# endernewton/tf-faster-rcnn

Hardware: NVIDIA H100
Metric: images/sec (higher is better)
Workload: dtype f16x3 (fp32-grade: fp16 hi/lo split of both operands, 3 wgmma f16 MMAs per product, fp32 accumulate)

## Files before the change

tf_faster_rcnn_b200/csrc/common.cuh:

```cuda
#pragma once
#include <cuda_runtime.h>
#include <cuda.h>
#include <stdint.h>
#include <stdio.h>

namespace frcnn {

enum Status : int {
  OK = 0, ERR_CUDA = -1, ERR_ARG = -2, ERR_NO_DEVICE = -3, ERR_DRIVER_ENTRY = -4, ERR_CAPACITY = -5
};
void set_error(const char* fmt, ...);
int cuda_fail(cudaError_t e, const char* what, const char* file, int line);

#define FRCNN_CUDA(expr)                                                        \
  do {                                                                          \
    cudaError_t _e = (expr);                                                    \
    if (_e != cudaSuccess) return ::frcnn::cuda_fail(_e, #expr, __FILE__, __LINE__); \
  } while (0)

#define FRCNN_LAUNCH_CHECK() FRCNN_CUDA(cudaGetLastError())

#define FRCNN_REQUIRE(cond, ...)                    \
  do {                                              \
    if (!(cond)) {                                  \
// ... 119 lines not shown
      "%32, %33, %34, %35, %36, %37, %38, %39, %40, %41, %42, %43, %44, %45, %46, %47, "
      "%48, %49, %50, %51, %52, %53, %54, %55, %56, %57, %58, %59, %60, %61, %62, %63}, "
      "{%64, %65, %66, %67}, %68, p, 1, 1, 0;\n\t}\n"
      : "+f"(d[0]), "+f"(d[1]), "+f"(d[2]), "+f"(d[3]), "+f"(d[4]), "+f"(d[5]), "+f"(d[6]), "+f"(d[7]),
        "+f"(d[8]), "+f"(d[9]), "+f"(d[10]), "+f"(d[11]), "+f"(d[12]), "+f"(d[13]), "+f"(d[14]), "+f"(d[15]),
        "+f"(d[16]), "+f"(d[17]), "+f"(d[18]), "+f"(d[19]), "+f"(d[20]), "+f"(d[21]), "+f"(d[22]), "+f"(d[23]),
        "+f"(d[24]), "+f"(d[25]), "+f"(d[26]), "+f"(d[27]), "+f"(d[28]), "+f"(d[29]), "+f"(d[30]), "+f"(d[31]),
        "+f"(d[32]), "+f"(d[33]), "+f"(d[34]), "+f"(d[35]), "+f"(d[36]), "+f"(d[37]), "+f"(d[38]), "+f"(d[39]),
        "+f"(d[40]), "+f"(d[41]), "+f"(d[42]), "+f"(d[43]), "+f"(d[44]), "+f"(d[45]), "+f"(d[46]), "+f"(d[47]),
        "+f"(d[48]), "+f"(d[49]), "+f"(d[50]), "+f"(d[51]), "+f"(d[52]), "+f"(d[53]), "+f"(d[54]), "+f"(d[55]),
        "+f"(d[56]), "+f"(d[57]), "+f"(d[58]), "+f"(d[59]), "+f"(d[60]), "+f"(d[61]), "+f"(d[62]), "+f"(d[63])
      : "r"(a[0]), "r"(a[1]), "r"(a[2]), "r"(a[3]), "l"(b_desc), "r"(scale_d));
}
template <> __device__ __forceinline__ void wgmma_tf32_rs<64>(float (&d)[32], const uint32_t (&a)[4], uint64_t b_desc, uint32_t scale_d) {
  asm volatile(
      "{\n\t.reg .pred p;\n\tsetp.ne.b32 p, %37, 0;\n\t"
      "wgmma.mma_async.sync.aligned.m64n64k8.f32.tf32.tf32 "
      "{%0, %1, %2, %3, %4, %5, %6, %7, %8, %9, %10, %11, %12, %13, %14, %15, "
      "%16, %17, %18, %19, %20, %21, %22, %23, %24, %25, %26, %27, %28, %29, %30, %31}, "
      "{%32, %33, %34, %35}, %36, p, 1, 1;\n\t}\n"
      : "+f"(d[0]), "+f"(d[1]), "+f"(d[2]), "+f"(d[3]), "+f"(d[4]), "+f"(d[5]), "+f"(d[6]), "+f"(d[7]),
        "+f"(d[8]), "+f"(d[9]), "+f"(d[10]), "+f"(d[11]), "+f"(d[12]), "+f"(d[13]), "+f"(d[14]), "+f"(d[15]),
        "+f"(d[16]), "+f"(d[17]), "+f"(d[18]), "+f"(d[19]), "+f"(d[20]), "+f"(d[21]), "+f"(d[22]), "+f"(d[23]),
        "+f"(d[24]), "+f"(d[25]), "+f"(d[26]), "+f"(d[27]), "+f"(d[28]), "+f"(d[29]), "+f"(d[30]), "+f"(d[31])
      : "r"(a[0]), "r"(a[1]), "r"(a[2]), "r"(a[3]), "l"(b_desc), "r"(scale_d));
}
template <> __device__ __forceinline__ void wgmma_tf32_rs<128>(float (&d)[64], const uint32_t (&a)[4], uint64_t b_desc, uint32_t scale_d) {
  asm volatile(
      "{\n\t.reg .pred p;\n\tsetp.ne.b32 p, %69, 0;\n\t"
      "wgmma.mma_async.sync.aligned.m64n128k8.f32.tf32.tf32 "
      "{%0, %1, %2, %3, %4, %5, %6, %7, %8, %9, %10, %11, %12, %13, %14, %15, "
      "%16, %17, %18, %19, %20, %21, %22, %23, %24, %25, %26, %27, %28, %29, %30, %31, "
      "%32, %33, %34, %35, %36, %37, %38, %39, %40, %41, %42, %43, %44, %45, %46, %47, "
      "%48, %49, %50, %51, %52, %53, %54, %55, %56, %57, %58, %59, %60, %61, %62, %63}, "
      "{%64, %65, %66, %67}, %68, p, 1, 1;\n\t}\n"
      : "+f"(d[0]), "+f"(d[1]), "+f"(d[2]), "+f"(d[3]), "+f"(d[4]), "+f"(d[5]), "+f"(d[6]), "+f"(d[7]),
        "+f"(d[8]), "+f"(d[9]), "+f"(d[10]), "+f"(d[11]), "+f"(d[12]), "+f"(d[13]), "+f"(d[14]), "+f"(d[15]),
        "+f"(d[16]), "+f"(d[17]), "+f"(d[18]), "+f"(d[19]), "+f"(d[20]), "+f"(d[21]), "+f"(d[22]), "+f"(d[23]),
        "+f"(d[24]), "+f"(d[25]), "+f"(d[26]), "+f"(d[27]), "+f"(d[28]), "+f"(d[29]), "+f"(d[30]), "+f"(d[31]),
        "+f"(d[32]), "+f"(d[33]), "+f"(d[34]), "+f"(d[35]), "+f"(d[36]), "+f"(d[37]), "+f"(d[38]), "+f"(d[39]),
        "+f"(d[40]), "+f"(d[41]), "+f"(d[42]), "+f"(d[43]), "+f"(d[44]), "+f"(d[45]), "+f"(d[46]), "+f"(d[47]),
        "+f"(d[48]), "+f"(d[49]), "+f"(d[50]), "+f"(d[51]), "+f"(d[52]), "+f"(d[53]), "+f"(d[54]), "+f"(d[55]),
        "+f"(d[56]), "+f"(d[57]), "+f"(d[58]), "+f"(d[59]), "+f"(d[60]), "+f"(d[61]), "+f"(d[62]), "+f"(d[63])
      : "r"(a[0]), "r"(a[1]), "r"(a[2]), "r"(a[3]), "l"(b_desc), "r"(scale_d));
}
template <int R> __device__ __forceinline__ void reg_dec() { asm volatile("setmaxnreg.dec.sync.aligned.u32 %0;" ::"n"(R)); }
template <int R> __device__ __forceinline__ void reg_inc() { asm volatile("setmaxnreg.inc.sync.aligned.u32 %0;" ::"n"(R)); }
__device__ __forceinline__ uint32_t pack_f16x2_rn(float a, float b) {
  uint32_t r;
  asm("cvt.rn.f16x2.f32 %0, %1, %2;" : "=r"(r) : "f"(b), "f"(a));
  return r;
}

__device__ __forceinline__ float4 ld_nc_f4_pinned(const float* p) {
  float4 v;
  asm volatile("ld.global.nc.v4.f32 {%0, %1, %2, %3}, [%4];" : "=f"(v.x), "=f"(v.y), "=f"(v.z), "=f"(v.w) : "l"(p));
  return v;
}
__device__ __forceinline__ float2 ld_nc_f2_pinned(const float* p) {
  float2 v;
  asm volatile("ld.global.nc.v2.f32 {%0, %1}, [%2];" : "=f"(v.x), "=f"(v.y) : "l"(p));
  return v;
}
__device__ __forceinline__ float2 ld_nc_f2_pinned_if(const float* p, bool pred) {
  float2 v = make_float2(0.f, 0.f);
  asm volatile("{\n\t.reg .pred q;\n\tsetp.ne.b32 q, %3, 0;\n\t@q ld.global.nc.v2.f32 {%0, %1}, [%2];\n\t}\n"
               : "+f"(v.x), "+f"(v.y) : "l"(p), "r"((int)pred));
  return v;
}
__device__ __forceinline__ float ld_nc_f32_pinned(const float* p) {
  float v;
  asm volatile("ld.global.nc.f32 %0, [%1];" : "=f"(v) : "l"(p));
  return v;
}

__device__ __forceinline__ float4 lds_f4(uint32_t saddr) {
  float4 v;
  asm volatile("ld.shared.v4.f32 {%0, %1, %2, %3}, [%4];" : "=f"(v.x), "=f"(v.y), "=f"(v.z), "=f"(v.w) : "r"(saddr));
  return v;
}

__device__ __forceinline__ void pdl_launch_dependents() { asm volatile("griddepcontrol.launch_dependents;" ::: "memory"); }
__device__ __forceinline__ void pdl_wait() { asm volatile("griddepcontrol.wait;" ::: "memory"); }

__device__ __forceinline__ float to_tf32_fast(float x) {
  return __uint_as_float((__float_as_uint(x) + 0x1000u) & 0xffffe000u);
}

__device__ __forceinline__ float to_tf32(float x) {
  uint32_t r;
  asm("cvt.rna.tf32.f32 %0, %1;" : "=r"(r) : "f"(x));
  return __uint_as_float(r);
}

#endif
}
```

tf_faster_rcnn_b200/csrc/conv_gemm.cu:

```cuda
#include <cuda_fp16.h>
#include "common.cuh"
#include "../../include/frcnn_b200.h"
#include <stdlib.h>
#include <string.h>

namespace frcnn {

constexpr int BLOCK_M = 128;
constexpr int BLOCK_K = 32;
constexpr int A_TILE_BYTES = BLOCK_M * BLOCK_K * 4;
constexpr int NUM_CONSUMERS = 256;
constexpr int NUM_THREADS = NUM_CONSUMERS + 128;
constexpr int REGS_PRODUCER = 40, REGS_CONSUMER = 232;
constexpr int STAGES = 3;

struct ConvKernelParams {
  float* out;
  const float* residual;
  const float* scale;
  const float* shift;
  int cout, ho, wo, nimg;
  int tn, th, tw;
  int tiles_h, tiles_w;
  int kh, kw, cin, stride, pad_t, pad_l;
  int act;
  int a_box_bytes;
  int kb_per_split;
  int m_tiles, n_tiles, total_units, n_full, splits;
  int raster_n;
  float* ws;
  long long* trace;
  int num_kb_total;
};

#ifdef FRCNN_WATCHDOG
#define FRCNN_TRACE(slot, kbv)                                                              \
  do {                                                                                      \
    if (p.trace && blockIdx.x == 0 && (kbv) < 64) p.trace[(kbv) * 8 + (slot)] = clock64(); \
  } while (0)
#else
#define FRCNN_TRACE(slot, kbv) do { } while (0)
#endif

template <int MODE> struct KTraits {
  static constexpr bool TF32 = MODE == FRCNN_CONV_TF32X3;
  static constexpr bool X1 = MODE == FRCNN_CONV_F16X1;
  static constexpr int BOXES = TF32 ? 1 : 2;
  static constexpr int A_BYTES = BOXES * A_TILE_BYTES;
  static constexpr float LO_SCALE = TF32 ? 1.f : 0.00048828125f;
};
template <int BN> constexpr int b_plane_bytes() { return BN * 128; }
template <int BN, int MODE> constexpr int stage_bytes() { return KTraits<MODE>::A_BYTES + 2 * b_plane_bytes<BN>(); }
template <int BN, int MODE> constexpr int smem_bytes() {
  return STAGES * stage_bytes<BN, MODE>() + 1024  + 64 ;
}
static_assert(smem_bytes<128, FRCNN_CONV_F16X3>() <= 227 * 1024, "ring exceeds the sm_90 shared-memory limit per block");

struct Unit {
  int w0, h0, n0, nblk, z, kb0, num_kb, slot;
};
__device__ __forceinline__ Unit decode_unit(const ConvKernelParams& p, int u, int num_kb_total) {
  Unit t;
  int tile;
  if (u < p.n_full) { tile = u; t.z = 0; t.slot = -1; }
  else { const int v = u - p.n_full; t.slot = v / p.splits; t.z = v - t.slot * p.splits; tile = p.n_full + t.slot; }
  int mt;
  if (p.raster_n) { t.nblk = tile % p.n_tiles; mt = tile / p.n_tiles; }
  else { mt = tile % p.m_tiles; t.nblk = tile / p.m_tiles; }
  const int tile_w = mt % p.tiles_w;
  const int tile_h = (mt / p.tiles_w) % p.tiles_h;
  const int tile_n = mt / (p.tiles_w * p.tiles_h);
  t.w0 = tile_w * p.tw; t.h0 = tile_h * p.th; t.n0 = tile_n * p.tn;
  if (t.slot < 0) { t.kb0 = 0; t.num_kb = num_kb_total; }
  else { t.kb0 = t.z * p.kb_per_split; t.num_kb = min(p.kb_per_split, num_kb_total - t.kb0); }
  return t;
}

template <int ACT>
__device__ __forceinline__ float apply_act(float a) {
  if (ACT == FRCNN_ACT_RELU) return fmaxf(a, 0.f);
  if (ACT == FRCNN_ACT_RELU6) return fminf(fmaxf(a, 0.f), 6.f);
  return a;
}

template <bool RES, int ACT>
__device__ __forceinline__ float2 finish2(const float2 v, const float2 sc, const float2 sh, const float2 r) {
  float2 y;
  y.x = __fadd_rn(__fmul_rn(v.x, sc.x), sh.x); y.y = __fadd_rn(__fmul_rn(v.y, sc.y), sh.y);
  if (RES) { y.x = __fadd_rn(y.x, r.x); y.y = __fadd_rn(y.y, r.y); }
  y.x = apply_act<ACT>(y.x); y.y = apply_act<ACT>(y.y);
  return y;
}

constexpr int EPI_CHUNK = 8;
template <int BN, bool RES, int ACT>
__device__ __forceinline__ void epilogue_vec(const ConvKernelParams& p, const float (&acc)[BN / 2], const int cbase,
                                             const int pix0, const int pix1) {
  const int cout = p.cout;
  constexpr int NJ = BN / 8;
  constexpr int CH = NJ < EPI_CHUNK ? NJ : EPI_CHUNK;
  static_assert(NJ % CH == 0, "chunking");
  const float* const res0 = RES ? p.residual + (size_t)(pix0 >= 0 ? pix0 : 0) * cout : nullptr;
  const float* const res1 = RES ? p.residual + (size_t)(pix1 >= 0 ? pix1 : 0) * cout : nullptr;
#pragma unroll
  for (int j0 = 0; j0 < NJ; j0 += CH) {
    if (cbase + 8 * j0 >= cout) break;
    float2 sc[CH], sh[CH], r0[CH], r1[CH];
#pragma unroll
    for (int jj = 0; jj < CH; ++jj) {
      const int c = cbase + 8 * (j0 + jj);
      sc[jj] = ld_nc_f2_pinned(p.scale + c);
      sh[jj] = ld_nc_f2_pinned(p.shift + c);
      if (RES) {
        r0[jj] = ld_nc_f2_pinned_if(res0 + c, pix0 >= 0 && c < cout);
        r1[jj] = ld_nc_f2_pinned_if(res1 + c, pix1 >= 0 && c < cout);
      } else {
        r0[jj] = r1[jj] = sc[jj];
      }
    }
#pragma unroll
    for (int jj = 0; jj < CH; ++jj) {
      const int j = j0 + jj;
      const int c = cbase + 8 * j;
      if (c >= cout) break;
      if (pix0 >= 0)
        *reinterpret_cast<float2*>(p.out + (size_t)pix0 * cout + c) =
            finish2<RES, ACT>(make_float2(acc[4 * j], acc[4 * j + 1]), sc[jj], sh[jj], r0[jj]);
      if (pix1 >= 0)
        *reinterpret_cast<float2*>(p.out + (size_t)pix1 * cout + c) =
            finish2<RES, ACT>(make_float2(acc[4 * j + 2], acc[4 * j + 3]), sc[jj], sh[jj], r1[jj]);
    }
  }
}

template <int BN>
__device__ __forceinline__ void epilogue_generic(const ConvKernelParams& p, const float (&acc)[BN / 2], const int cbase,
                                                 const int pix0, const int pix1) {
#pragma unroll
  for (int j = 0; j < BN / 8; ++j) {
#pragma unroll
    for (int e = 0; e < 4; ++e) {
      const int c = cbase + 8 * j + (e & 1);
      const int pix = e < 2 ? pix0 : pix1;
      if (pix < 0 || c >= p.cout) continue;
      float a = __fadd_rn(__fmul_rn(acc[4 * j + e], p.scale[c]), p.shift[c]);
      if (p.residual) a = __fadd_rn(a, __ldg(p.residual + (size_t)pix * p.cout + c));
      if (p.act == FRCNN_ACT_RELU) a = fmaxf(a, 0.f);
      else if (p.act == FRCNN_ACT_RELU6) a = fminf(fmaxf(a, 0.f), 6.f);
      p.out[(size_t)pix * p.cout + c] = a;
    }
  }
}

template <int BN, bool RES>
__device__ __forceinline__ void epilogue_dispatch(const ConvKernelParams& p, const float (&acc)[BN / 2], const int cbase,
                                                  const int pix0, const int pix1) {
  if (p.act == FRCNN_ACT_RELU) epilogue_vec<BN, RES, FRCNN_ACT_RELU>(p, acc, cbase, pix0, pix1);
  else if (p.act == FRCNN_ACT_RELU6) epilogue_vec<BN, RES, FRCNN_ACT_RELU6>(p, acc, cbase, pix0, pix1);
  else epilogue_vec<BN, RES, FRCNN_ACT_NONE>(p, acc, cbase, pix0, pix1);
}

__device__ __forceinline__ int tile_pixel(const ConvKernelParams& p, const Unit& t, int row) {
  const int rows_img = p.th * p.tw;
  const int dn = row / rows_img, rem = row % rows_img;
  const int n = t.n0 + dn, h = t.h0 + rem / p.tw, w = t.w0 + rem % p.tw;
  const bool valid = row < p.tn * rows_img && n < p.nimg && h < p.ho && w < p.wo;
  return valid ? (int)(((long long)n * p.ho + h) * p.wo + w) : -1;
}

template <int BN>
__device__ __forceinline__ void epilogue_tile(const ConvKernelParams& p, const Unit& t, const float (&acc)[BN / 2], int r0, int q4) {
  if (t.slot >= 0) {
    float* const w = p.ws + ((size_t)t.slot * p.splits + t.z) * (size_t)(BLOCK_M * BN) + 2 * q4;
#pragma unroll
    for (int j = 0; j < BN / 8; ++j) {
      __stcg(reinterpret_cast<float2*>(w + (size_t)r0 * BN + 8 * j), make_float2(acc[4 * j], acc[4 * j + 1]));
      __stcg(reinterpret_cast<float2*>(w + (size_t)(r0 + 8) * BN + 8 * j), make_float2(acc[4 * j + 2], acc[4 * j + 3]));
    }
    return;
  }
  const int pix0 = tile_pixel(p, t, r0), pix1 = tile_pixel(p, t, r0 + 8);
  const int cbase = t.nblk * BN + 2 * q4;
  if ((p.cout & 3) != 0) {
    epilogue_generic<BN>(p, acc, cbase, pix0, pix1);
    return;
  }
  if (p.residual) epilogue_dispatch<BN, true>(p, acc, cbase, pix0, pix1);
  else epilogue_dispatch<BN, false>(p, acc, cbase, pix0, pix1);
}

template <int BN, int MODE>
__device__ __forceinline__ void wgmma_rs(float (&d)[BN / 2], const uint32_t (&a)[4], uint64_t b_desc, uint32_t scale_d) {
  if (KTraits<MODE>::TF32) wgmma_tf32_rs<BN>(d, a, b_desc, scale_d);
  else wgmma_f16_rs<BN>(d, a, b_desc, scale_d);
}

template <int BN, int MODE>
__global__ void __launch_bounds__(NUM_THREADS, 1)
conv_gemm_kernel(const __grid_constant__ CUtensorMap tmA, const __grid_constant__ CUtensorMap tmBhi,
                 const __grid_constant__ CUtensorMap tmBlo, const ConvKernelParams p) {
  using T = KTraits<MODE>;
  constexpr int kStage = stage_bytes<BN, MODE>();
  constexpr int kPlane = b_plane_bytes<BN>();
  constexpr int NACC = BN / 2;
  static_assert(BN == 64 || BN == 128, "block_n");

  extern __shared__ uint8_t smem_raw[];
  uint8_t* smem = reinterpret_cast<uint8_t*>((reinterpret_cast<uintptr_t>(smem_raw) + 1023) & ~uintptr_t(1023));
  uint64_t* full = reinterpret_cast<uint64_t*>(smem + STAGES * kStage);
  uint64_t* empty = full + STAGES;

  const int warp = threadIdx.x >> 5;
  const int lane = threadIdx.x & 31;
  const int num_kb_total = p.num_kb_total;

  if (threadIdx.x == NUM_CONSUMERS) {
    tma_prefetch_desc(&tmA); tma_prefetch_desc(&tmBhi); tma_prefetch_desc(&tmBlo);
    for (int s = 0; s < STAGES; ++s) { mbar_init(&full[s], 1); mbar_init(&empty[s], NUM_CONSUMERS); }
    mbar_fence_init();
  }
  __syncthreads();
  pdl_launch_dependents();
  pdl_wait();

  if (warp >= NUM_CONSUMERS / 32) {
    reg_dec<REGS_PRODUCER>();
    if (warp == NUM_CONSUMERS / 32 && lane == 0) {
      const int cchunks = p.cin / BLOCK_K;
      const int total32 = p.kh * p.kw * cchunks;
      const uint32_t tx = (uint32_t)(T::BOXES * p.a_box_bytes + (T::X1 ? 1 : 2) * kPlane);
      int s = 0; uint32_t ph = 0, kbt = 0;
      for (int u = blockIdx.x; u < p.total_units; u += gridDim.x) {
        const Unit t = decode_unit(p, u, num_kb_total);
#pragma unroll 1
        for (int kb = 0; kb < t.num_kb; ++kb, ++kbt) {
          MBAR_WAIT(&empty[s], ph ^ 1u, 4, kbt);
          uint8_t* st = smem + s * kStage;
          mbar_expect_tx(&full[s], tx);
#pragma unroll
          for (int i = 0; i < T::BOXES; ++i) {
            const int g32 = (t.kb0 + kb) * T::BOXES + i;
            int tap = g32 / cchunks, kc = g32 - tap * cchunks;
            if (g32 >= total32) { tap = 0; kc = cchunks; }
            const int r = tap / p.kw, sx = tap - r * p.kw;
            tma_load_4d(st + i * A_TILE_BYTES, &tmA, &full[s], kc * BLOCK_K, t.w0 * p.stride + sx - p.pad_l,
                        t.h0 * p.stride + r - p.pad_t, t.n0);
          }
          const int kcoord = (t.kb0 + kb) * T::BOXES * BLOCK_K;
          tma_load_2d(st + T::A_BYTES, &tmBhi, &full[s], kcoord, t.nblk * BN);
          if (!T::X1) tma_load_2d(st + T::A_BYTES + kPlane, &tmBlo, &full[s], kcoord, t.nblk * BN);
          FRCNN_TRACE(0, kbt);
          if (++s == STAGES) { s = 0; ph ^= 1u; }
        }
      }
    }
    return;
  }

  reg_inc<REGS_CONSUMER>();
  const int wg = warp >> 2;
  const int q4 = lane & 3;
  const int r0 = wg * 64 + (warp & 3) * 16 + (lane >> 2);
  const uint32_t swz = (uint32_t)(lane >> 2);
  uint32_t aoff[4][2];
#pragma unroll
  for (int j = 0; j < 4; ++j)
#pragma unroll
    for (int h = 0; h < 2; ++h) {
      const int ch = T::TF32 ? j * 8 + h * 4 + q4 : (j & 1) * 16 + h * 8 + 2 * q4;
      const int box = T::TF32 ? 0 : j >> 1;
      aoff[j][h] = (uint32_t)(box * A_TILE_BYTES + r0 * 128) + ((((uint32_t)ch >> 2) ^ swz) << 4) + (((uint32_t)ch & 3u) << 2);
    }
  const uint32_t smem0 = smem_u32(smem);
  int s = 0; uint32_t ph = 0, kbt = 0;
  for (int u = blockIdx.x; u < p.total_units; u += gridDim.x) {
    const Unit t = decode_unit(p, u, num_kb_total);
    float acc[NACC], part[NACC];
#pragma unroll
    for (int i = 0; i < NACC; ++i) { acc[i] = 0.f; part[i] = 0.f; }
#pragma unroll 1
    for (int kb = 0; kb < t.num_kb; ++kb, ++kbt) {
      MBAR_WAIT(&full[s], ph, 1, kbt);
      if (threadIdx.x == 0) FRCNN_TRACE(1, kbt);
      const uint32_t sa = smem0 + (uint32_t)(s * kStage);
      uint32_t ahi[4][4], alo[4][4];
#pragma unroll
      for (int j = 0; j < 4; ++j) {
#pragma unroll
        for (int f = 0; f < 4; ++f) {
          const uint32_t addr = sa + aoff[j][f >> 1] + ((f & 1) ? 1024u : 0u);
          if (T::TF32) {
            float x;
            asm volatile("ld.shared.f32 %0, [%1];" : "=f"(x) : "r"(addr));
            const float hi = to_tf32(x);
            ahi[j][f] = __float_as_uint(hi);
            alo[j][f] = __float_as_uint(to_tf32_fast(__fsub_rn(x, hi)));
          } else {
            float2 x;
            asm volatile("ld.shared.v2.f32 {%0, %1}, [%2];" : "=f"(x.x), "=f"(x.y) : "r"(addr));
            const uint32_t h = pack_f16x2_rn(x.x, x.y);
            const float2 fh = __half22float2(*reinterpret_cast<const __half2*>(&h));
            ahi[j][f] = h;
            alo[j][f] = T::X1 ? 0u : pack_f16x2_rn(__fmul_rn(__fsub_rn(x.x, fh.x), 2048.f), __fmul_rn(__fsub_rn(x.y, fh.y), 2048.f));
          }
        }
      }
      const uint64_t bhi = wgmma_sw128_desc(sa + (uint32_t)T::A_BYTES);
      const uint64_t blo = wgmma_sw128_desc(sa + (uint32_t)(T::A_BYTES + kPlane));
#pragma unroll
      for (int i = 0; i < NACC; ++i) reg_fence(part[i]);
      wgmma_fence();
#pragma unroll
      for (int j = 0; j < 4; ++j) wgmma_rs<BN, MODE>(part, ahi[j], bhi + 2u * j, j > 0 ? 1u : 0u);
      wgmma_commit();
      wgmma_wait_all();
#pragma unroll
      for (int i = 0; i < NACC; ++i) { reg_fence(part[i]); acc[i] = __fadd_rn(acc[i], part[i]); }
      if (!T::X1) {
        wgmma_fence();
#pragma unroll
        for (int j = 0; j < 4; ++j) {
          wgmma_rs<BN, MODE>(part, alo[j], bhi + 2u * j, j > 0 ? 1u : 0u);
          wgmma_rs<BN, MODE>(part, ahi[j], blo + 2u * j, 1u);
        }
        wgmma_commit();
        wgmma_wait_all();
#pragma unroll
        for (int i = 0; i < NACC; ++i) { reg_fence(part[i]); acc[i] = __fmaf_rn(part[i], T::LO_SCALE, acc[i]); }
      }
      mbar_arrive(&empty[s]);
      if (threadIdx.x == 0) FRCNN_TRACE(2, kbt);
      if (++s == STAGES) { s = 0; ph ^= 1u; }
    }
    epilogue_tile<BN>(p, t, acc, r0, q4);
  }
}

template <int BN>
__global__ void __launch_bounds__(256)
tail_reduce_kernel(const ConvKernelParams p) {
  pdl_launch_dependents();
  pdl_wait();
  constexpr int RPB = 256 / (BN / 4);
  constexpr int GROUPS = BLOCK_M / RPB;
  const int slot = blockIdx.x / GROUPS, rgroup = blockIdx.x % GROUPS;
  const int tile = p.n_full + slot;
  const int mt = p.raster_n ? tile / p.n_tiles : tile % p.m_tiles, nblk = p.raster_n ? tile % p.n_tiles : tile / p.m_tiles;
  const int tile_w = mt % p.tiles_w, tile_h = (mt / p.tiles_w) % p.tiles_h, tile_n = mt / (p.tiles_w * p.tiles_h);
  const int rows_img = p.th * p.tw;
  constexpr int C4 = BN / 4;
  static_assert(256 % C4 == 0, "each thread keeps one fixed channel group");
  const float* base = p.ws + (size_t)slot * p.splits * (size_t)(BLOCK_M * BN);
  const bool vec_ok = (p.cout & 3) == 0;
  const int cg = threadIdx.x % C4;
  const int c = nblk * BN + cg * 4;
  if (c >= p.cout) return;
  const float4 sc4 = __ldg(reinterpret_cast<const float4*>(p.scale + c)), sh4 = __ldg(reinterpret_cast<const float4*>(p.shift + c));
  const float sc[4] = {sc4.x, sc4.y, sc4.z, sc4.w}, sh[4] = {sh4.x, sh4.y, sh4.z, sh4.w};
  {
    const int row = rgroup * RPB + threadIdx.x / C4;
    const int dn = row / rows_img, rem = row % rows_img;
    const int n = tile_n * p.tn + dn, h = tile_h * p.th + rem / p.tw, w = tile_w * p.tw + rem % p.tw;
    if (row >= p.tn * rows_img || n >= p.nimg || h >= p.ho || w >= p.wo) return;
    const size_t o = ((((size_t)n * p.ho + h) * p.wo + w)) * p.cout + c;
    float4 rv = make_float4(0.f, 0.f, 0.f, 0.f);
    if (p.residual) {
      if (vec_ok) rv = __ldg(reinterpret_cast<const float4*>(p.residual + o));
      else { float t[4] = {0.f, 0.f, 0.f, 0.f}; for (int e = 0; e < 4; ++e) if (c + e < p.cout) t[e] = __ldg(p.residual + o + e); rv = make_float4(t[0], t[1], t[2], t[3]); }
    }
    float4 a = __ldg(reinterpret_cast<const float4*>(base + (size_t)row * BN) + cg);
    for (int z = 1; z < p.splits; ++z) {
      const float4 b = __ldg(reinterpret_cast<const float4*>(base + ((size_t)z * BLOCK_M + row) * BN) + cg);
      a.x = __fadd_rn(a.x, b.x); a.y = __fadd_rn(a.y, b.y); a.z = __fadd_rn(a.z, b.z); a.w = __fadd_rn(a.w, b.w);
    }
    float y[4] = {a.x, a.y, a.z, a.w};
    const float res[4] = {rv.x, rv.y, rv.z, rv.w};
#pragma unroll
    for (int e = 0; e < 4; ++e) {
      float v = y[e];
      v = __fadd_rn(__fmul_rn(v, sc[e]), sh[e]);
      if (p.residual) v = __fadd_rn(v, res[e]);
      if (p.act == FRCNN_ACT_RELU) v = fmaxf(v, 0.f);
      else if (p.act == FRCNN_ACT_RELU6) v = fminf(fmaxf(v, 0.f), 6.f);
      y[e] = v;
    }
    if (vec_ok) *reinterpret_cast<float4*>(p.out + o) = make_float4(y[0], y[1], y[2], y[3]);
    else for (int e = 0; e < 4; ++e) if (c + e < p.cout) p.out[o + e] = y[e];
// ... 1 lines not shown
}

__global__ void prep_epilogue_vectors_kernel(const float* scale, const float* shift, float out_mult, int cout, int padded,
                                             float* eff_scale, float* eff_shift) {
  const int c = blockIdx.x * blockDim.x + threadIdx.x;
  if (c >= padded) return;
  const float sc = (c < cout && scale) ? scale[c] : 1.f;
  eff_scale[c] = __fmul_rn(sc, out_mult);
  eff_shift[c] = (c < cout && shift) ? shift[c] : 0.f;
}

typedef CUresult (*EncodeTiledFn)(CUtensorMap*, CUtensorMapDataType, cuuint32_t, void*, const cuuint64_t*,
                                  const cuuint64_t*, const cuuint32_t*, const cuuint32_t*, CUtensorMapInterleave,
                                  CUtensorMapSwizzle, CUtensorMapL2promotion, CUtensorMapFloatOOBfill);

static EncodeTiledFn get_encode_fn() {
  static EncodeTiledFn fn = nullptr;
  if (!fn) {
    void* ptr = nullptr;
    cudaDriverEntryPointQueryResult qres;
    if (cudaGetDriverEntryPoint("cuTensorMapEncodeTiled", &ptr, cudaEnableDefault, &qres) == cudaSuccess &&
        qres == cudaDriverEntryPointSuccess)
      fn = reinterpret_cast<EncodeTiledFn>(ptr);
  }
  return fn;
}

static int encode_map(CUtensorMap* m, const void* base, int rank, const uint64_t* dims, const uint64_t* strides_bytes,
                      const uint32_t* box, const uint32_t* estr, CUtensorMapDataType dtype = CU_TENSOR_MAP_DATA_TYPE_FLOAT32,
                      CUtensorMapSwizzle swz = CU_TENSOR_MAP_SWIZZLE_128B) {
  EncodeTiledFn fn = get_encode_fn();
  if (!fn) { set_error("cuTensorMapEncodeTiled entry point unavailable"); return ERR_DRIVER_ENTRY; }
  cuuint64_t gd[5]; cuuint64_t gs[4]; cuuint32_t bx[5]; cuuint32_t es[5];
  for (int i = 0; i < rank; ++i) { gd[i] = dims[i]; bx[i] = box[i]; es[i] = estr[i]; }
  for (int i = 0; i + 1 < rank; ++i) gs[i] = strides_bytes[i];
  CUresult r = fn(m, dtype, (cuuint32_t)rank, const_cast<void*>(base), gd, gs, bx, es,
                  CU_TENSOR_MAP_INTERLEAVE_NONE, swz, CU_TENSOR_MAP_L2_PROMOTION_L2_256B,
                  CU_TENSOR_MAP_FLOAT_OOB_FILL_NONE);
  if (r != CUDA_SUCCESS) {
    set_error("cuTensorMapEncodeTiled failed (CUresult %d) rank=%d dims=[%llu,%llu,%llu,%llu] box=[%u,%u,%u,%u]", (int)r, rank,
              (unsigned long long)dims[0], (unsigned long long)dims[1], rank > 2 ? (unsigned long long)dims[2] : 0ull,
              rank > 3 ? (unsigned long long)dims[3] : 0ull, box[0], box[1], rank > 2 ? box[2] : 0u, rank > 3 ? box[3] : 0u);
    return ERR_CUDA;
  }
  return OK;
}

}

using namespace frcnn;

struct frcnn_conv_plan {
  CUtensorMap tmA, tmBhi, tmBlo;
  ConvKernelParams kp;
  int block_n, stages, smem;
  int impl;
  dim3 grid;
  int n_tail;
  float* ws;
  float* eff;
};

static void choose_tile(int n, int ho, int wo, int stride, int* tn, int* th, int* tw) {
  long best_tiles = -1; int bn = 1, bh = 1, bw = 1; int best_rows = 0;
  const int lim = 256 / stride;
  for (int a = 1; a <= n && a <= BLOCK_M; ++a)
    for (int b = 1; b <= ho && a * b <= BLOCK_M && b <= lim; ++b) {
      int c = BLOCK_M / (a * b);
      if (c > wo) c = wo;
      if (c > lim) c = lim;
      if (c < 1) continue;
      int tiles_w = cdiv(wo, c);
      c = cdiv(wo, tiles_w);
      long tiles = (long)cdiv(n, a) * cdiv(ho, b) * tiles_w;
      int rows = a * b * c;
      if (best_tiles < 0 || tiles < best_tiles || (tiles == best_tiles && rows < best_rows)) {
        best_tiles = tiles; bn = a; bh = b; bw = c; best_rows = rows;
      }
    }
  *tn = bn; *th = bh; *tw = bw;
}

static bool pdl_enabled() {
  static int v = -1;
  if (v < 0) { const char* e = getenv("FRCNN_NO_PDL"); v = (e && e[0] == '1') ? 0 : 1; }
  return v == 1;
}

template <int BN, int MODE>
static int launch(const frcnn_conv_plan* p, cudaStream_t st) {
  static bool attr_done = false;
  if (!attr_done) {
    FRCNN_CUDA(cudaFuncSetAttribute(conv_gemm_kernel<BN, MODE>, cudaFuncAttributeMaxDynamicSharedMemorySize, smem_bytes<BN, MODE>()));
    attr_done = true;
  }
  cudaLaunchAttribute attr[1];
  attr[0].id = cudaLaunchAttributeProgrammaticStreamSerialization;
  attr[0].val.programmaticStreamSerializationAllowed = 1;
  const bool pdl = pdl_enabled();
  cudaLaunchConfig_t cfg{};
  cfg.gridDim = p->grid; cfg.blockDim = dim3(NUM_THREADS); cfg.dynamicSmemBytes = smem_bytes<BN, MODE>(); cfg.stream = st;
  cfg.attrs = attr; cfg.numAttrs = pdl ? 1 : 0;
  FRCNN_CUDA(cudaLaunchKernelEx(&cfg, conv_gemm_kernel<BN, MODE>, p->tmA, p->tmBhi, p->tmBlo, p->kp));
  if (p->n_tail > 0) {
    cudaLaunchConfig_t rc{};
    rc.gridDim = dim3((unsigned)(p->n_tail * (BLOCK_M / (256 / (BN / 4))))); rc.blockDim = dim3(256); rc.dynamicSmemBytes = 0; rc.stream = st;
    rc.attrs = attr; rc.numAttrs = pdl ? 1 : 0;
    FRCNN_CUDA(cudaLaunchKernelEx(&rc, tail_reduce_kernel<BN>, p->kp));
  }
  return OK;
}

struct Geometry {
  int n, h, w, ho, wo;
  int tn, th, tw, tiles_w, tiles_h, tiles_n;
  long m_tiles;
  int num_kb, bn, n_tiles, kpc;
  long tiles, n_tail;
  int splits, kbs;
  long total_units;
  int grid;
  int raster_n;
};

static int decide_geometry(const frcnn_conv_desc* d, int sms, Geometry* g) {
  FRCNN_REQUIRE(d->cin > 0 && d->cin % BLOCK_K == 0, "cin=%d must be a positive multiple of 32", d->cin);
  FRCNN_REQUIRE(d->kh >= 1 && d->kw >= 1 && d->stride >= 1 && d->stride <= 8, "bad filter geometry");
  FRCNN_REQUIRE(d->n > 0 && d->h > 0 && d->w > 0 && d->ho > 0 && d->wo > 0 && d->cout > 0, "bad shape");
  FRCNN_REQUIRE(sms > 0, "bad SM count");
  g->n = d->n; g->h = d->h; g->w = d->w; g->ho = d->ho; g->wo = d->wo;
  const bool pointwise = d->kh == 1 && d->kw == 1 && d->stride == 1 && d->pad_t == 0 && d->pad_l == 0 && g->ho == g->h && g->wo == g->w;
  if (pointwise) {
    g->w = g->wo = g->n * g->h * g->w; g->n = 1; g->h = g->ho = 1;
  }
  choose_tile(g->n, g->ho, g->wo, d->stride, &g->tn, &g->th, &g->tw);
  g->tiles_w = cdiv(g->wo, g->tw); g->tiles_h = cdiv(g->ho, g->th); g->tiles_n = cdiv(g->n, g->tn);
  g->m_tiles = (long)g->tiles_w * g->tiles_h * g->tiles_n;
  const bool f16 = d->impl != FRCNN_CONV_TF32X3;
  const int ks = f16 ? 2 : 1;
  g->num_kb = cdiv(d->kh * d->kw * d->cin / BLOCK_K, ks);
  g->kpc = d->kb_per_chunk > 0 ? d->kb_per_chunk : 8 / ks;
  int bn = d->block_n;
  if (bn == 0) {
    long best = -1;
    const int cands[2] = {128, 64};
    for (int i = 0; i < 2; ++i) {
      const int c = cands[i];
      if (c > 64 && c / 2 >= d->cout) continue;
      const long ctas = g->m_tiles * cdiv(d->cout, c);
      const long waves = (ctas + sms - 1) / sms;
      const long cost = f16 ? waves * (g->num_kb * 900L + 4000L) : waves * (g->num_kb * 1400L + 6000L);
      if (best < 0 || cost < best) { best = cost; bn = c; }
    }
  }
  FRCNN_REQUIRE(bn == 64 || bn == 128, "block_n must be 64 or 128");
  g->bn = bn;
// ... 20 lines not shown
  g->total_units = (g->tiles - n_tail) + n_tail * splits;
  FRCNN_REQUIRE(g->total_units <= 0x7fffffffL, "too many work units");
  g->grid = (int)(g->total_units < sms ? g->total_units : sms);
  {
    const char* e = getenv("FRCNN_CONV_RASTER");
    const double a_bytes = (double)d->n * d->h * d->w * d->cin * 4.0, b_bytes = (double)d->cout * d->kh * d->kw * d->cin * 4.0;
    g->raster_n = (e && (e[0] == 'm' || e[0] == 'n')) ? (e[0] == 'n') : (a_bytes > b_bytes && g->n_tiles > 1);
  }
  return OK;
}

extern "C" int frcnn_conv_plan_geometry(const frcnn_conv_desc* d, int sm_count, int* out16) {
  FRCNN_REQUIRE(d && out16, "null argument");
  Geometry g;
  int rc = decide_geometry(d, sm_count, &g);
  if (rc) return rc;
  const int v[16] = {g.bn, g.tn, g.th, g.tw, (int)g.m_tiles, g.n_tiles, (int)g.tiles, (int)g.n_tail, g.splits, g.kbs,
                     (int)g.total_units, g.grid, g.num_kb, g.kpc, g.tiles_h, g.tiles_w};
  for (int i = 0; i < 16; ++i) out16[i] = v[i];
  return OK;
}

extern "C" int frcnn_conv_plan_create(frcnn_conv_plan** out, const frcnn_conv_desc* d) {
  FRCNN_REQUIRE(out && d, "null argument");
  FRCNN_REQUIRE(d->in_dev && d->w_hi_dev && d->w_lo_dev && d->out_dev, "null device pointer");
  int sms = 132;
  { int dev = 0; cudaDeviceProp pr; if (cudaGetDevice(&dev) == cudaSuccess && cudaGetDeviceProperties(&pr, dev) == cudaSuccess && pr.multiProcessorCount > 0) sms = pr.multiProcessorCount; }
  Geometry g;
  int grc = decide_geometry(d, sms, &g);
  if (grc) return grc;
  frcnn_conv_plan* p = (frcnn_conv_plan*)aligned_alloc(64, (sizeof(frcnn_conv_plan) + 63) / 64 * 64);
  if (!p) { set_error("out of host memory"); return ERR_ARG; }
  memset(p, 0, sizeof(*p));
  const int bn = g.bn;
  {
    uint64_t dims[4] = {(uint64_t)d->cin, (uint64_t)g.w, (uint64_t)g.h, (uint64_t)g.n};
    uint64_t strides[3] = {(uint64_t)d->cin * 4, (uint64_t)g.w * d->cin * 4, (uint64_t)g.h * g.w * d->cin * 4};
    uint32_t box[4] = {(uint32_t)BLOCK_K, (uint32_t)(g.tw * d->stride), (uint32_t)(g.th * d->stride), (uint32_t)g.tn};
    uint32_t es[4] = {1, (uint32_t)d->stride, (uint32_t)d->stride, 1};
    int rc = encode_map(&p->tmA, d->in_dev, 4, dims, strides, box, es);
    if (rc) { free(p); return rc; }
  }
  const bool f16 = d->impl != FRCNN_CONV_TF32X3;
  {
    const uint64_t ktot = (uint64_t)d->kh * d->kw * d->cin;
    uint64_t dims[2] = {ktot, (uint64_t)d->cout};
    uint64_t strides[1] = {ktot * (f16 ? 2 : 4)};
    uint32_t box[2] = {(uint32_t)(f16 ? 2 * BLOCK_K : BLOCK_K), (uint32_t)bn};
    uint32_t es[2] = {1, 1};
    const CUtensorMapDataType dt = f16 ? CU_TENSOR_MAP_DATA_TYPE_FLOAT16 : CU_TENSOR_MAP_DATA_TYPE_FLOAT32;
    const CUtensorMapSwizzle sw = CU_TENSOR_MAP_SWIZZLE_128B;
    int rc = encode_map(&p->tmBhi, d->w_hi_dev, 2, dims, strides, box, es, dt, sw);
    if (!rc) rc = encode_map(&p->tmBlo, d->w_lo_dev, 2, dims, strides, box, es, dt, sw);
    if (rc) { free(p); return rc; }
  }
  ConvKernelParams& k = p->kp;
  k.out = d->out_dev; k.residual = d->residual_dev;
  k.cout = d->cout; k.ho = g.ho; k.wo = g.wo; k.nimg = g.n;
  k.tn = g.tn; k.th = g.th; k.tw = g.tw; k.tiles_h = g.tiles_h; k.tiles_w = g.tiles_w;
  k.kh = d->kh; k.kw = d->kw; k.cin = d->cin; k.stride = d->stride; k.pad_t = d->pad_t; k.pad_l = d->pad_l;
  k.act = d->act;
  k.a_box_bytes = g.tn * g.th * g.tw * BLOCK_K * 4;
  k.trace = nullptr;
  k.num_kb_total = g.num_kb;
  k.m_tiles = (int)g.m_tiles; k.n_tiles = g.n_tiles;
  k.kb_per_split = g.kbs; k.splits = g.splits; k.n_full = (int)(g.tiles - g.n_tail);
  k.total_units = (int)g.total_units;
  k.raster_n = g.raster_n;
  k.ws = nullptr; p->ws = nullptr; p->eff = nullptr; p->n_tail = (int)g.n_tail;
  {
    const int padded = g.n_tiles * bn;
    const float om = f16 ? (d->out_mult != 0.f ? d->out_mult : 1.f) : 1.f;
    cudaError_t e = cudaMalloc(&p->eff, (size_t)2 * padded * sizeof(float));
    if (e != cudaSuccess) { free(p); return cuda_fail(e, "epilogue vectors", __FILE__, __LINE__); }
    prep_epilogue_vectors_kernel<<<cdiv(padded, 256), 256>>>(d->scale_dev, d->shift_dev, om, d->cout, padded, p->eff, p->eff + padded);
    e = cudaGetLastError();
    if (e == cudaSuccess) e = cudaDeviceSynchronize();
    if (e != cudaSuccess) { cudaFree(p->eff); free(p); return cuda_fail(e, "prep_epilogue_vectors", __FILE__, __LINE__); }
    k.scale = p->eff; k.shift = p->eff + padded;
  }
  if (g.n_tail > 0) {
    cudaError_t e = cudaMalloc(&p->ws, (size_t)g.n_tail * g.splits * BLOCK_M * bn * sizeof(float));
    if (e != cudaSuccess) { cudaFree(p->eff); free(p); return cuda_fail(e, "split-tile workspace", __FILE__, __LINE__); }
    k.ws = p->ws;
  }
  p->grid = dim3((unsigned)g.grid, 1, 1);
  p->block_n = bn;
  p->impl = f16 ? (d->impl == FRCNN_CONV_F16X1 ? FRCNN_CONV_F16X1 : FRCNN_CONV_F16X3) : FRCNN_CONV_TF32X3;
  p->stages = STAGES;
  p->smem = f16 ? (bn == 128 ? smem_bytes<128, FRCNN_CONV_F16X3>() : smem_bytes<64, FRCNN_CONV_F16X3>())
              : (bn == 128 ? smem_bytes<128, FRCNN_CONV_TF32X3>() : smem_bytes<64, FRCNN_CONV_TF32X3>());
  *out = p;
  return OK;
}

extern "C" int frcnn_conv_plan_run(const frcnn_conv_plan* p, void* stream) {
  FRCNN_REQUIRE(p, "null plan");
  cudaStream_t st = (cudaStream_t)stream;
  if (p->impl == FRCNN_CONV_F16X3) return p->block_n == 128 ? launch<128, FRCNN_CONV_F16X3>(p, st) : launch<64, FRCNN_CONV_F16X3>(p, st);
  if (p->impl == FRCNN_CONV_F16X1) return p->block_n == 128 ? launch<128, FRCNN_CONV_F16X1>(p, st) : launch<64, FRCNN_CONV_F16X1>(p, st);
  return p->block_n == 128 ? launch<128, FRCNN_CONV_TF32X3>(p, st) : launch<64, FRCNN_CONV_TF32X3>(p, st);
}

extern "C" int frcnn_conv_plan_info(const frcnn_conv_plan* p, int* block_n, int* tile_n, int* tile_h, int* tile_w,
                                    int* grid_m, int* grid_n, int* stages, int* smem) {
  FRCNN_REQUIRE(p, "null plan");
// ... 37 lines not shown
```

Measured before the change: 257.2.

## Stage epilogue through shared memory with TMA residual loads and tensor stores

Replaces the per-thread global epilogue (scale/shift/residual loads and float2 stores) with a dedicated storer warp. It prefetches residual tiles and scale/shift vectors into double-buffered shared-memory slots via TMA/bulk copies, then writes finished 32-column chunks back with TMA tensor stores. Consumers apply the affine, residual and activation in shared memory and signal the storer through named barriers. The aim is to cut uncoalesced global traffic and overlap output writes with the next tile's MMA, at the cost of extra shared memory and added synchronisation.

```diff
diff --git a/tf_faster_rcnn_b200/csrc/common.cuh b/tf_faster_rcnn_b200/csrc/common.cuh
--- a/tf_faster_rcnn_b200/csrc/common.cuh
+++ b/tf_faster_rcnn_b200/csrc/common.cuh
@@ -195,32 +195,35 @@
   return r;
 }
 
-__device__ __forceinline__ float4 ld_nc_f4_pinned(const float* p) {
-  float4 v;
-  asm volatile("ld.global.nc.v4.f32 {%0, %1, %2, %3}, [%4];" : "=f"(v.x), "=f"(v.y), "=f"(v.z), "=f"(v.w) : "l"(p));
+__device__ __forceinline__ void tma_store_4d(const CUtensorMap* m, const void* src, int c0, int c1, int c2, int c3) {
+  asm volatile(
+      "cp.async.bulk.tensor.4d.global.shared::cta.tile.bulk_group [%0, {%2, %3, %4, %5}], [%1];"
+      ::"l"(reinterpret_cast<uint64_t>(m)), "r"(smem_u32(src)), "r"(c0), "r"(c1), "r"(c2), "r"(c3)
+      : "memory");
+}
+__device__ __forceinline__ void bulk_commit() { asm volatile("cp.async.bulk.commit_group;" ::: "memory"); }
+__device__ __forceinline__ void bulk_wait_read_all() { asm volatile("cp.async.bulk.wait_group.read 0;" ::: "memory"); }
+__device__ __forceinline__ void bulk_wait_all() { asm volatile("cp.async.bulk.wait_group 0;" ::: "memory"); }
+__device__ __forceinline__ void bulk_load(void* dst, const void* src, uint32_t bytes, uint64_t* bar) {
+  asm volatile("cp.async.bulk.shared::cluster.global.mbarrier::complete_tx::bytes [%0], [%1], %2, [%3];"
+               ::"r"(smem_u32(dst)), "l"(reinterpret_cast<uint64_t>(src)), "r"(bytes), "r"(smem_u32(bar))
+               : "memory");
+}
+__device__ __forceinline__ void fence_proxy_async_smem() { asm volatile("fence.proxy.async.shared::cta;" ::: "memory"); }
+__device__ __forceinline__ void named_bar_arrive(uint32_t id, uint32_t count) {
+  asm volatile("bar.arrive %0, %1;" ::"r"(id), "r"(count) : "memory");
+}
+__device__ __forceinline__ void named_bar_sync(uint32_t id, uint32_t count) {
+  asm volatile("bar.sync %0, %1;" ::"r"(id), "r"(count) : "memory");
+}
+
+__device__ __forceinline__ float2 lds_f2(uint32_t saddr) {
+  float2 v;
+  asm volatile("ld.shared.v2.f32 {%0, %1}, [%2];" : "=f"(v.x), "=f"(v.y) : "r"(saddr));
   return v;
 }
-__device__ __forceinline__ float2 ld_nc_f2_pinned(const float* p) {
-  float2 v;
-  asm volatile("ld.global.nc.v2.f32 {%0, %1}, [%2];" : "=f"(v.x), "=f"(v.y) : "l"(p));
-  return v;
-}
-__device__ __forceinline__ float2 ld_nc_f2_pinned_if(const float* p, bool pred) {
-  float2 v = make_float2(0.f, 0.f);
-  asm volatile("{\n\t.reg .pred q;\n\tsetp.ne.b32 q, %3, 0;\n\t@q ld.global.nc.v2.f32 {%0, %1}, [%2];\n\t}\n"
-               : "+f"(v.x), "+f"(v.y) : "l"(p), "r"((int)pred));
-  return v;
-}
-__device__ __forceinline__ float ld_nc_f32_pinned(const float* p) {
-  float v;
-  asm volatile("ld.global.nc.f32 %0, [%1];" : "=f"(v) : "l"(p));
-  return v;
-}
-
-__device__ __forceinline__ float4 lds_f4(uint32_t saddr) {
-  float4 v;
-  asm volatile("ld.shared.v4.f32 {%0, %1, %2, %3}, [%4];" : "=f"(v.x), "=f"(v.y), "=f"(v.z), "=f"(v.w) : "r"(saddr));
-  return v;
+__device__ __forceinline__ void sts_f2(uint32_t saddr, float2 v) {
+  asm volatile("st.shared.v2.f32 [%0], {%1, %2};" ::"r"(saddr), "f"(v.x), "f"(v.y) : "memory");
 }
 
 __device__ __forceinline__ void pdl_launch_dependents() { asm volatile("griddepcontrol.launch_dependents;" ::: "memory"); }
diff --git a/tf_faster_rcnn_b200/csrc/conv_gemm.cu b/tf_faster_rcnn_b200/csrc/conv_gemm.cu
--- a/tf_faster_rcnn_b200/csrc/conv_gemm.cu
+++ b/tf_faster_rcnn_b200/csrc/conv_gemm.cu
@@ -51,10 +51,15 @@
 };
 template <int BN> constexpr int b_plane_bytes() { return BN * 128; }
 template <int BN, int MODE> constexpr int stage_bytes() { return KTraits<MODE>::A_BYTES + 2 * b_plane_bytes<BN>(); }
+constexpr int EPI_COLS = 32;
+constexpr int EPI_SLOT_BYTES = BLOCK_M * EPI_COLS * 4;
+constexpr int EPI_VEC_BYTES = 2 * EPI_COLS * 4;
+constexpr int EPI_SLOTS = 2;
+constexpr int BAR_BYTES = (2 * STAGES + EPI_SLOTS) * 8;
 template <int BN, int MODE> constexpr int smem_bytes() {
-  return STAGES * stage_bytes<BN, MODE>() + 1024  + 64 ;
-}
-static_assert(smem_bytes<128, FRCNN_CONV_F16X3>() <= 227 * 1024, "ring exceeds the sm_90 shared-memory limit per block");
+  return STAGES * stage_bytes<BN, MODE>() + EPI_SLOTS * (EPI_SLOT_BYTES + EPI_VEC_BYTES) + 1024  + BAR_BYTES;
+}
+static_assert(smem_bytes<128, FRCNN_CONV_F16X3>() <= 227 * 1024, "ring + staging slots exceed the sm_90 shared-memory limit per block");
 
 struct Unit {
   int w0, h0, n0, nblk, z, kb0, num_kb, slot;
@@ -92,44 +97,66 @@
   return y;
 }
 
-constexpr int EPI_CHUNK = 8;
+template <int BN>
+__device__ __forceinline__ int epi_chunks(const ConvKernelParams& p, const Unit& t) {
+  if (t.slot >= 0 || (p.cout & 3) != 0) return 0;
+  const int n = (p.cout - t.nblk * BN + EPI_COLS - 1) / EPI_COLS;
+  return n < BN / EPI_COLS ? n : BN / EPI_COLS;
+}
+
+struct ChunkPos {
+  int u, c, n, col, w0, h0, n0;
+};
+template <int BN>
+__device__ __forceinline__ void chunk_next(const ConvKernelParams& p, ChunkPos& k) {
+  if (++k.c < k.n) { k.col += EPI_COLS; return; }
+  k.c = 0;
+  for (k.u += gridDim.x; k.u < p.total_units; k.u += gridDim.x) {
+    const Unit t = decode_unit(p, k.u, p.num_kb_total);
+    k.n = epi_chunks<BN>(p, t);
+    k.col = t.nblk * BN; k.w0 = t.w0; k.h0 = t.h0; k.n0 = t.n0;
+    if (k.n > 0) return;
+  }
+}
+template <int BN>
+__device__ __forceinline__ ChunkPos chunk_first(const ConvKernelParams& p) {
+  ChunkPos k;
+  k.u = (int)blockIdx.x - (int)gridDim.x; k.c = 0; k.n = 0; k.col = k.w0 = k.h0 = k.n0 = 0;
+  chunk_next<BN>(p, k);
+  return k;
+}
+
+__device__ __forceinline__ void epi_load(const ConvKernelParams& p, const CUtensorMap* tmRes, uint8_t* slot, uint8_t* vec,
+                                         uint64_t* landed, const ChunkPos& k) {
+  mbar_expect_tx(landed, (uint32_t)(EPI_VEC_BYTES + (p.residual ? p.a_box_bytes : 0)));
+  bulk_load(vec, p.scale + k.col, EPI_COLS * 4, landed);
+  bulk_load(vec + EPI_COLS * 4, p.shift + k.col, EPI_COLS * 4, landed);
+  if (p.residual) tma_load_4d(slot, tmRes, landed, k.col, k.w0, k.h0, k.n0);
+}
+
 template <int BN, bool RES, int ACT>
-__device__ __forceinline__ void epilogue_vec(const ConvKernelParams& p, const float (&acc)[BN / 2], const int cbase,
-                                             const int pix0, const int pix1) {
-  const int cout = p.cout;
-  constexpr int NJ = BN / 8;
-  constexpr int CH = NJ < EPI_CHUNK ? NJ : EPI_CHUNK;
-  static_assert(NJ % CH == 0, "chunking");
-  const float* const res0 = RES ? p.residual + (size_t)(pix0 >= 0 ? pix0 : 0) * cout : nullptr;
-  const float* const res1 = RES ? p.residual + (size_t)(pix1 >= 0 ? pix1 : 0) * cout : nullptr;
-#pragma unroll
-  for (int j0 = 0; j0 < NJ; j0 += CH) {
-    if (cbase + 8 * j0 >= cout) break;
-    float2 sc[CH], sh[CH], r0[CH], r1[CH];
-#pragma unroll
-    for (int jj = 0; jj < CH; ++jj) {
-      const int c = cbase + 8 * (j0 + jj);
-      sc[jj] = ld_nc_f2_pinned(p.scale + c);
-      sh[jj] = ld_nc_f2_pinned(p.shift + c);
-      if (RES) {
-        r0[jj] = ld_nc_f2_pinned_if(res0 + c, pix0 >= 0 && c < cout);
-        r1[jj] = ld_nc_f2_pinned_if(res1 + c, pix1 >= 0 && c < cout);
-      } else {
-        r0[jj] = r1[jj] = sc[jj];
-      }
-    }
-#pragma unroll
-    for (int jj = 0; jj < CH; ++jj) {
-      const int j = j0 + jj;
-      const int c = cbase + 8 * j;
-      if (c >= cout) break;
-      if (pix0 >= 0)
-        *reinterpret_cast<float2*>(p.out + (size_t)pix0 * cout + c) =
-            finish2<RES, ACT>(make_float2(acc[4 * j], acc[4 * j + 1]), sc[jj], sh[jj], r0[jj]);
-      if (pix1 >= 0)
-        *reinterpret_cast<float2*>(p.out + (size_t)pix1 * cout + c) =
-            finish2<RES, ACT>(make_float2(acc[4 * j + 2], acc[4 * j + 3]), sc[jj], sh[jj], r1[jj]);
-    }
+__device__ __forceinline__ void epilogue_chunks(const float (&acc)[BN / 2], const int n, uint32_t& q, uint64_t* landed,
+                                                const uint32_t slot0, const uint32_t vec0, const int r0, const int q4) {
+  const uint32_t swz = (uint32_t)(r0 & 7);
+#pragma unroll
+  for (int c = 0; c < BN / EPI_COLS; ++c) {
+    if (c >= n) break;
+    const uint32_t i = q % EPI_SLOTS;
+    MBAR_WAIT(&landed[i], (q / EPI_SLOTS) & 1u, 5, q);
+    const uint32_t sb = slot0 + i * EPI_SLOT_BYTES + (uint32_t)r0 * 128u, vb = vec0 + i * EPI_VEC_BYTES;
+#pragma unroll
+    for (int jj = 0; jj < EPI_COLS / 8; ++jj) {
+      const int j = c * (EPI_COLS / 8) + jj;
+      const uint32_t col = 8u * jj + 2u * q4;
+      const uint32_t a0 = sb + ((((col >> 2) ^ swz) << 4) | ((col & 3u) << 2));
+      const float2 sc = lds_f2(vb + 4u * col), sh = lds_f2(vb + 4u * (EPI_COLS + col));
+      const float2 res0 = RES ? lds_f2(a0) : sc, res1 = RES ? lds_f2(a0 + 1024u) : sc;
+      sts_f2(a0, finish2<RES, ACT>(make_float2(acc[4 * j], acc[4 * j + 1]), sc, sh, res0));
+      sts_f2(a0 + 1024u, finish2<RES, ACT>(make_float2(acc[4 * j + 2], acc[4 * j + 3]), sc, sh, res1));
+    }
+    fence_proxy_async_smem();
+    named_bar_arrive(1 + i, NUM_CONSUMERS + 32);
+    ++q;
   }
 }
 
@@ -152,14 +179,6 @@
   }
 }
 
-template <int BN, bool RES>
-__device__ __forceinline__ void epilogue_dispatch(const ConvKernelParams& p, const float (&acc)[BN / 2], const int cbase,
-                                                  const int pix0, const int pix1) {
-  if (p.act == FRCNN_ACT_RELU) epilogue_vec<BN, RES, FRCNN_ACT_RELU>(p, acc, cbase, pix0, pix1);
-  else if (p.act == FRCNN_ACT_RELU6) epilogue_vec<BN, RES, FRCNN_ACT_RELU6>(p, acc, cbase, pix0, pix1);
-  else epilogue_vec<BN, RES, FRCNN_ACT_NONE>(p, acc, cbase, pix0, pix1);
-}
-
 __device__ __forceinline__ int tile_pixel(const ConvKernelParams& p, const Unit& t, int row) {
   const int rows_img = p.th * p.tw;
   const int dn = row / rows_img, rem = row % rows_img;
@@ -169,7 +188,23 @@
 }
 
 template <int BN>
-__device__ __forceinline__ void epilogue_tile(const ConvKernelParams& p, const Unit& t, const float (&acc)[BN / 2], int r0, int q4) {
+__device__ __forceinline__ void epilogue_tile(const ConvKernelParams& p, const Unit& t, const float (&acc)[BN / 2], int r0, int q4,
+                                              uint32_t& q, uint64_t* landed, uint32_t slot0, uint32_t vec0) {
+  const int n = epi_chunks<BN>(p, t);
+  if (n > 0) {
+#define FRCNN_EPI_CHUNKS(RES, ACT) epilogue_chunks<BN, RES, ACT>(acc, n, q, landed, slot0, vec0, r0, q4)
+    if (p.residual) {
+      if (p.act == FRCNN_ACT_RELU) FRCNN_EPI_CHUNKS(true, FRCNN_ACT_RELU);
+      else if (p.act == FRCNN_ACT_RELU6) FRCNN_EPI_CHUNKS(true, FRCNN_ACT_RELU6);
+      else FRCNN_EPI_CHUNKS(true, FRCNN_ACT_NONE);
+    } else {
+      if (p.act == FRCNN_ACT_RELU) FRCNN_EPI_CHUNKS(false, FRCNN_ACT_RELU);
+      else if (p.act == FRCNN_ACT_RELU6) FRCNN_EPI_CHUNKS(false, FRCNN_ACT_RELU6);
+      else FRCNN_EPI_CHUNKS(false, FRCNN_ACT_NONE);
+    }
+#undef FRCNN_EPI_CHUNKS
+    return;
+  }
   if (t.slot >= 0) {
     float* const w = p.ws + ((size_t)t.slot * p.splits + t.z) * (size_t)(BLOCK_M * BN) + 2 * q4;
 #pragma unroll
@@ -179,14 +214,7 @@
     }
     return;
   }
-  const int pix0 = tile_pixel(p, t, r0), pix1 = tile_pixel(p, t, r0 + 8);
-  const int cbase = t.nblk * BN + 2 * q4;
-  if ((p.cout & 3) != 0) {
-    epilogue_generic<BN>(p, acc, cbase, pix0, pix1);
-    return;
-  }
-  if (p.residual) epilogue_dispatch<BN, true>(p, acc, cbase, pix0, pix1);
-  else epilogue_dispatch<BN, false>(p, acc, cbase, pix0, pix1);
+  epilogue_generic<BN>(p, acc, t.nblk * BN + 2 * q4, tile_pixel(p, t, r0), tile_pixel(p, t, r0 + 8));
 }
 
 template <int BN, int MODE>
@@ -198,17 +226,22 @@
 template <int BN, int MODE>
 __global__ void __launch_bounds__(NUM_THREADS, 1)
 conv_gemm_kernel(const __grid_constant__ CUtensorMap tmA, const __grid_constant__ CUtensorMap tmBhi,
-                 const __grid_constant__ CUtensorMap tmBlo, const ConvKernelParams p) {
+                 const __grid_constant__ CUtensorMap tmBlo, const __grid_constant__ CUtensorMap tmOut,
+                 const __grid_constant__ CUtensorMap tmRes, const ConvKernelParams p) {
   using T = KTraits<MODE>;
   constexpr int kStage = stage_bytes<BN, MODE>();
   constexpr int kPlane = b_plane_bytes<BN>();
   constexpr int NACC = BN / 2;
   static_assert(BN == 64 || BN == 128, "block_n");
+  static_assert(BN % EPI_COLS == 0, "epilogue chunks");
 
   extern __shared__ uint8_t smem_raw[];
   uint8_t* smem = reinterpret_cast<uint8_t*>((reinterpret_cast<uintptr_t>(smem_raw) + 1023) & ~uintptr_t(1023));
-  uint64_t* full = reinterpret_cast<uint64_t*>(smem + STAGES * kStage);
+  uint8_t* slots = smem + STAGES * kStage;
+  uint8_t* vecs = slots + EPI_SLOTS * EPI_SLOT_BYTES;
+  uint64_t* full = reinterpret_cast<uint64_t*>(vecs + EPI_SLOTS * EPI_VEC_BYTES);
   uint64_t* empty = full + STAGES;
+  uint64_t* landed = empty + STAGES;
 
   const int warp = threadIdx.x >> 5;
   const int lane = threadIdx.x & 31;
@@ -217,6 +250,7 @@
   if (threadIdx.x == NUM_CONSUMERS) {
     tma_prefetch_desc(&tmA); tma_prefetch_desc(&tmBhi); tma_prefetch_desc(&tmBlo);
     for (int s = 0; s < STAGES; ++s) { mbar_init(&full[s], 1); mbar_init(&empty[s], NUM_CONSUMERS); }
+    for (int i = 0; i < EPI_SLOTS; ++i) mbar_init(&landed[i], 1);
     mbar_fence_init();
   }
   __syncthreads();
@@ -253,6 +287,27 @@
           if (++s == STAGES) { s = 0; ph ^= 1u; }
         }
       }
+    } else if (warp == NUM_CONSUMERS / 32 + 1) {
+      ChunkPos ld = chunk_first<BN>(p);
+      if (lane == 0 && ld.u < p.total_units) { tma_prefetch_desc(&tmOut); if (p.residual) tma_prefetch_desc(&tmRes); }
+      for (int i = 0; i < EPI_SLOTS && ld.u < p.total_units; ++i, chunk_next<BN>(p, ld))
+        if (lane == 0) epi_load(p, &tmRes, slots + i * EPI_SLOT_BYTES, vecs + i * EPI_VEC_BYTES, &landed[i], ld);
+      uint32_t q = 0;
+      for (ChunkPos st = chunk_first<BN>(p); st.u < p.total_units; chunk_next<BN>(p, st), ++q) {
+        const uint32_t i = q % EPI_SLOTS;
+        __syncwarp();
+        named_bar_sync(1 + i, NUM_CONSUMERS + 32);
+        if (lane == 0) {
+          tma_store_4d(&tmOut, slots + i * EPI_SLOT_BYTES, st.col, st.w0, st.h0, st.n0);
+          bulk_commit();
+          if (ld.u < p.total_units) {
+            bulk_wait_read_all();
+            epi_load(p, &tmRes, slots + i * EPI_SLOT_BYTES, vecs + i * EPI_VEC_BYTES, &landed[i], ld);
+          }
+        }
+        if (ld.u < p.total_units) chunk_next<BN>(p, ld);
+      }
+      if (lane == 0) bulk_wait_all();
     }
     return;
   }
@@ -273,6 +328,7 @@
     }
   const uint32_t smem0 = smem_u32(smem);
   int s = 0; uint32_t ph = 0, kbt = 0;
+  uint32_t q = 0;
   for (int u = blockIdx.x; u < p.total_units; u += gridDim.x) {
     const Unit t = decode_unit(p, u, num_kb_total);
     float acc[NACC], part[NACC];
@@ -332,7 +388,7 @@
       if (threadIdx.x == 0) FRCNN_TRACE(2, kbt);
       if (++s == STAGES) { s = 0; ph ^= 1u; }
     }
-    epilogue_tile<BN>(p, t, acc, r0, q4);
+    epilogue_tile<BN>(p, t, acc, r0, q4, q, landed, smem_u32(slots), smem_u32(vecs));
   }
 }
 
@@ -440,6 +496,7 @@
 
 struct frcnn_conv_plan {
   CUtensorMap tmA, tmBhi, tmBlo;
+  CUtensorMap tmOut, tmRes;
   ConvKernelParams kp;
   int block_n, stages, smem;
   int impl;
@@ -489,7 +546,7 @@
   cudaLaunchConfig_t cfg{};
   cfg.gridDim = p->grid; cfg.blockDim = dim3(NUM_THREADS); cfg.dynamicSmemBytes = smem_bytes<BN, MODE>(); cfg.stream = st;
   cfg.attrs = attr; cfg.numAttrs = pdl ? 1 : 0;
-  FRCNN_CUDA(cudaLaunchKernelEx(&cfg, conv_gemm_kernel<BN, MODE>, p->tmA, p->tmBhi, p->tmBlo, p->kp));
+  FRCNN_CUDA(cudaLaunchKernelEx(&cfg, conv_gemm_kernel<BN, MODE>, p->tmA, p->tmBhi, p->tmBlo, p->tmOut, p->tmRes, p->kp));
   if (p->n_tail > 0) {
     cudaLaunchConfig_t rc{};
     rc.gridDim = dim3((unsigned)(p->n_tail * (BLOCK_M / (256 / (BN / 4))))); rc.blockDim = dim3(256); rc.dynamicSmemBytes = 0; rc.stream = st;
@@ -616,6 +673,15 @@
     const CUtensorMapSwizzle sw = CU_TENSOR_MAP_SWIZZLE_128B;
     int rc = encode_map(&p->tmBhi, d->w_hi_dev, 2, dims, strides, box, es, dt, sw);
     if (!rc) rc = encode_map(&p->tmBlo, d->w_lo_dev, 2, dims, strides, box, es, dt, sw);
+    if (rc) { free(p); return rc; }
+  }
+  if ((d->cout & 3) == 0) {
+    uint64_t dims[4] = {(uint64_t)d->cout, (uint64_t)g.wo, (uint64_t)g.ho, (uint64_t)g.n};
+    uint64_t strides[3] = {(uint64_t)d->cout * 4, (uint64_t)g.wo * d->cout * 4, (uint64_t)g.ho * g.wo * d->cout * 4};
+    uint32_t box[4] = {(uint32_t)EPI_COLS, (uint32_t)g.tw, (uint32_t)g.th, (uint32_t)g.tn};
+    uint32_t es[4] = {1, 1, 1, 1};
+    int rc = encode_map(&p->tmOut, d->out_dev, 4, dims, strides, box, es);
+    if (!rc && d->residual_dev) rc = encode_map(&p->tmRes, d->residual_dev, 4, dims, strides, box, es);
     if (rc) { free(p); return rc; }
   }
   ConvKernelParams& k = p->kp;
```

New measurement: 264.7, median of 6. +2.9%, better.
